# chenruduan/OAReactDiff

Hardware: AMD Instinct MI355X
Metric: denoising_steps_per_sec (higher is better)
Workload: dtype f32; 1 GPU; EGNNDynamics.forward (LEFTNet H=196 R=96 L=6), B=64 reactions/GPU x 3 objects x 23 atoms, complete graph per reaction (N=4416, E=300288), T=1000 sampler step shape; batch_per_gpu=64, atoms_per_object=23, parallelism=replica x1 (no collective), launch=eager

## Files before the change

### oareactdiff_amd/_capi.py

```python
from __future__ import annotations

import ctypes as C
import os

from .build import LIB

OARD_MAX_OBJECTS = 8
ABI_VERSION = 2040
OARD_OK, OARD_EINVAL, OARD_ENOTCOMPLETE, OARD_EHIP, OARD_ENOMEM = 0, -1, -2, -3, -4
ERRORS = {OARD_EINVAL: "invalid argument / unsupported configuration", OARD_ENOTCOMPLETE: "topology is not complete-per-sample",
          OARD_EHIP: "HIP runtime error", OARD_ENOMEM: "workspace too small"}

PREC_GCL_BF16X3, PREC_EQUI_BF16X3, PREC_TRAIN_BF16X3 = 1, 2, 4
TAP_S, TAP_VEC, TAP_EDGE, TAP_POS_FRAME, TAP_DPOS, TAP_HOUT, TAP_LABELS, TAP_NE1 = 1, 2, 3, 4, 5, 6, 7, 8

EXPORTS = ["oard_version", "oard_supported", "oard_param_count", "oard_packed_bytes", "oard_pack_weights",
           "oard_topology_create", "oard_topology_destroy", "oard_topology_num_nodes", "oard_topology_num_edges",
           "oard_topology_num_inner_edges", "oard_topology_num_samples", "oard_topology_check_edge_index",
           "oard_workspace_bytes", "oard_forward", "oard_active_inner_edges", "oard_debug_lin3u_table", "oard_sampler_step", "oard_sampler_step_dev", "oard_tap", "oard_debug_stop_after", "oard_debug_option", "oard_timing_enable", "oard_timing_reset",
           "oard_timing_get",
           "oard_topology_create_parts", "oard_topology_export", "oard_tape_bytes", "oard_tape_entry", "oard_forward_train",
           "oard_packed_bwd_bytes", "oard_pack_weights_bwd", "oard_gcl_backward_dx", "oard_edge_node_sums",
           "oard_equi_backward_dx", "oard_scalarize_backward", "oard_equi_msg_backward", "oard_lin3u_forward", "oard_lin3u_backward", "oard_wgrad_scratch_bytes", "oard_wgrad",
           "oard_train_scratch_bytes", "oard_train_scratch_poison", "oard_train_scratch_entry", "oard_train_tail_backward",
# ... 106 lines not shown
    L.oard_train_stage_backward.restype = ci
    L.oard_nan_replace.argtypes = [cfgp, vp, vp, pvp, pvp, vp]; L.oard_nan_replace.restype = ci
    pf, cf = C.POINTER(C.c_float), C.c_float
    L.oard_loss_prepare.argtypes = [cfgp, vp, pvp, pvp, pvp, pvp, vp, vp, ci, pf, pf, ci, ci, pvp, pvp, vp]; L.oard_loss_prepare.restype = ci
    L.oard_loss_terms.argtypes = [cfgp, vp, pvp, pvp, pvp, pvp, pvp, vp, vp, ci, pf, pf, pf, ci, ci, vp, vp, pvp, vp]; L.oard_loss_terms.restype = ci
    cd = C.c_double
    L.oard_adamw_step.argtypes = [vp, vp, vp, vp, vp, i64, cd, cd, cd, cd, cd, i64, ci, cd, vp]; L.oard_adamw_step.restype = ci
    L.oard_adamw_step_dev.argtypes = [vp, vp, vp, vp, vp, i64, cd, cd, cd, cd, cd, ci, ci, vp, ci, vp, vp, vp, vp]; L.oard_adamw_step_dev.restype = ci
    L.oard_library_stream.argtypes = [ci, pvp]; L.oard_library_stream.restype = ci
    L.oard_graph_create.argtypes = [cfgp, vp, vp, i64, vp, i64, pvp]; L.oard_graph_create.restype = ci
    L.oard_graph_destroy.argtypes = [vp]; L.oard_graph_destroy.restype = None
    L.oard_graph_num_nodes.argtypes = [vp]; L.oard_graph_num_nodes.restype = i64
    L.oard_graph_num_edges.argtypes = [vp]; L.oard_graph_num_edges.restype = i64
    L.oard_graph_object_rows.argtypes = [vp, ci]; L.oard_graph_object_rows.restype = i64
    L.oard_graph_is_complete.argtypes = [vp]; L.oard_graph_is_complete.restype = ci
    L.oard_graph_workspace_bytes.argtypes = [cfgp, vp]; L.oard_graph_workspace_bytes.restype = sz
    L.oard_graph_forward.argtypes = [cfgp, vp, pvp, sz, pvp, vp, ci, vp, pvp, vp, sz, vp, vp]; L.oard_graph_forward.restype = ci
    L.oard_debug_stop_after.argtypes = [C.c_int]; L.oard_debug_stop_after.restype = C.c_int
    L.oard_debug_option.argtypes = [C.c_char_p, C.c_int]; L.oard_debug_option.restype = C.c_int
    L.oard_timing_enable.argtypes = [C.c_int]; L.oard_timing_enable.restype = C.c_int
    L.oard_timing_reset.argtypes = []; L.oard_timing_reset.restype = C.c_int
    L.oard_timing_get.argtypes = [C.c_char_p, C.POINTER(C.c_double), C.POINTER(i64)]; L.oard_timing_get.restype = C.c_int
    for env, opt in (("OARD_GCL_VARIANT", b"gcl_variant"), ("OARD_EQUI_VARIANT", b"equi_variant"),
                     ("OARD_NODE_VARIANT", b"node_variant"), ("OARD_GCL_SKIP", b"gcl_skip"), ("OARD_EQUI_SKIP", b"equi_skip"), ("OARD_EQUI_L0_SKIP", b"equi_l0_skip"), ("OARD_GCL_MSUM", b"gcl_msum"), ("OARD_GCL_PERSIST", b"gcl_persist"), ("OARD_GCL_GRID", b"gcl_grid"), ("OARD_PARTS", b"parts"), ("OARD_SEQUENTIAL", b"sequential"), ("OARD_POISON", b"poison"), ("OARD_AUTO_SMALL", b"auto_small"), ("OARD_AUTO_TINY", b"auto_tiny"), ("OARD_NPB", b"npb"),
                     ("OARD_WGRAD_WGS", b"wgrad_wgs"), ("OARD_WGRAD_LDS", b"wgrad_lds"), ("OARD_WGRAD_T16", b"wgrad_t16"), ("OARD_WGRAD_QUEUE", b"wgrad_queue"), ("OARD_GATE_FOLD", b"gate_fold"), ("OARD_WGRAD_SHAPES", b"wgrad_shapes"), ("OARD_TRAIN_DUAL", b"train_dual"), ("OARD_SMALL_SPLIT", b"small_split"),
                     ("OARD_SKIP_FAMILIES", b"skip_families")):
        if os.environ.get(env) not in (None, ""):
            check(L.oard_debug_option(opt, int(os.environ[env])), f"oard_debug_option({opt.decode()})")
    _lib = L
    return L


def timing_get(family: str):
    ms, n = C.c_double(0.0), C.c_int64(0)
    check(lib().oard_timing_get(family.encode(), C.byref(ms), C.byref(n)), "oard_timing_get")
    return ms.value, n.value
```

### oareactdiff_amd/csrc/oard_hip.hip

```cpp
#include <algorithm>
#include <cmath>
#include <cstdio>
#include <cstring>
#include <map>
#include <string>
#include <vector>
#include <mutex>
#include <chrono>
#include <utility>

#include "oard_kernels.h"
#include "oard_edge_v1.h"
#include "oard_edge_p.h"
#include "oard_wgrad_t16.h"
#include "oard_edge_b3.h"
#ifdef OARD_EXPERIMENTS
#include "oard_edge_fp.h"
#endif
#include "oard_node_v1.h"
#include "oard_edge_small.h"
#include "oard_edge_bwd.h"
#include "oard_node_bwd.h"
#include "oard_rows.h"
#include "oard_inst.h"
// ... 24 lines not shown
        hipEvent_t e; (void)hipEventCreate(&e); return e;
    }
    void flush() {
        for (auto& r : recs) {
            (void)hipEventSynchronize(r.b);
            float ms = 0.f;
            (void)hipEventElapsedTime(&ms, r.a, r.b);
            total_ms[r.fam] += ms; launches[r.fam] += 1;
            pool.push_back(r.a); pool.push_back(r.b);
        }
        recs.clear();
    }
} g_timing;
int g_stop_after = 0;
int g_gcl_variant = 2;
int g_equi_variant = 2;
int g_sequential = 0;
int g_auto_tiny = 8;
int g_auto_small = 4;
int g_npb = 0;
int g_poison = 0;
int g_equi_l0_skip = 1;
int g_gcl_msum = 1;
int g_gcl_msum_taken = 0;
int g_equi_l0_taken = 0;
int g_parts = 0;
int g_small_split = 128;
int g_wgrad_shapes = 3;
int g_wgrad_t16 = 256;
int g_wgrad_lds = 256;
int g_wgrad_wgs = 512;
int g_gcl_persist = 1;
int g_gcl_grid = 0;
int g_equi_skip = 1;
int g_gcl_skip = 1;
int g_node_variant = 1;
int g_skip_families = 0;

struct ScopedLaunch {
    hipStream_t st; hipEvent_t a; int fam; bool on;
    ScopedLaunch(int f, hipStream_t s) : st(s), fam(f), on(g_timing.on) {
        if (on) { a = g_timing.get(); (void)hipEventRecord(a, st); }
    }
    ~ScopedLaunch() {
        if (on) { hipEvent_t b = g_timing.get(); (void)hipEventRecord(b, st); g_timing.recs.push_back({a, b, fam}); }
    }
// ... 198 lines not shown
static thread_local SmallScratch t_small = {nullptr, nullptr};
static WsOff make_ws(const oard_config* c, const TopoDev& td) {
    const RDims d(c->hidden, c->num_radial);
    const size_t N = td.N, E = td.E + 1, A = td.A + 1;
    WsOff w;
    size_t cur = 0;
    auto take = [&](size_t bytes) { size_t o = cur; cur = align_up(cur + bytes, 256); return o; };
    w.pos = take(N * 3 * 4); w.pf64 = take(N * 3 * 8); w.pf32 = take(N * 3 * 4); w.x1 = take(N * 3 * 4);
    w.pp0 = take(N * 4); w.labels = take(N * 4); w.hin = take(N * 16 * 4);
    w.zemb = take(N * d.HP * 4); w.nb = take(N * d.HP * 4); w.s = take(N * d.HP * 4); w.s1 = take(N * d.HP * 4);
    w.ne1 = take(N * 3 * d.HP * 4); w.xh = take(N * d.HP * 4); w.P = take(N * d.HP * 4); w.Q = take(N * d.HP * 4);
    w.xq = take(N * 3 * d.HP * 4); w.vec = take(N * 3 * d.HP * 4); w.vec2 = take(N * 3 * d.HP * 4); w.v2buf = take(N * 3 * d.HP * 4);
    w.sc0 = take(N * d.HP * 4); w.vdot = take(N * d.HP * 4);
    w.geo = take(A * GEO_STRIDE * 4); w.d64 = take(A * 8); w.rbuf = take(A * d.RP * 4);
    w.ew = take(E * d.WP * 4); w.mbuf = take(std::max(E, (size_t)(td.CI + td.CX) + 1) * d.HP * 4);
    w.xmsg = take(A * d.HP * 4); w.vmsg = take(A * 3 * d.HP * 4);
    w.dpos = take(N * 3 * 4); w.hout = take(N * 16 * 4);
    w.al_rows = take(A * 4); w.al_src = take(A * 4); w.al_pre = take(A * 4); w.al_cnt = take((size_t)cdiv((long long)td.A, 256) * 4 + 4); w.al_n = take(4);
    w.d1s = take((size_t)cdiv((long long)td.A, 128) * 8 * d.D1T * 1024);
    w.small_a = w.small_b = 0;
    if (E <= (size_t)OARD_SMALL_MAX_EDGES) {
        w.small_a = take(A * d.D1P * 4);
    }
    w.total = cur;
    return w;
}



template <class K>
int set_lds(K kernel, size_t bytes) {
    HIP_TRY(hipFuncSetAttribute((const void*)kernel, hipFuncAttributeMaxDynamicSharedMemorySize, (int)bytes));
    return OARD_OK;
}

#define LAUNCH_LDS(fam, kern, grid, block, lds, stream, ...) do { \
    static bool attr_done_[64] = {}; \
    int dev_ = 0; (void)hipGetDevice(&dev_); dev_ &= 63; \
    if (!attr_done_[dev_]) { int rc_ = set_lds(kern, lds); if (rc_ != OARD_OK) return rc_; attr_done_[dev_] = true; } \
    ScopedLaunch sl_(fam, stream); if (!((g_skip_families >> (fam)) & 1)) \
    hipLaunchKernelGGL(kern, dim3((unsigned)(grid)), dim3(block), lds, stream, __VA_ARGS__); } while (0)

#define GCL_CASE(id, WV_, GP_) case id: { \
        LAUNCH_LDS(F_GCL_EDGE, (k_gcl_edge_v1<D, WV_, GP_, S1, S3, false>), cdiv(r1 - r0, 16 * WV_), WV_ * 64, \
                   (GclStream<D, GP_>::LDS_BYTES), st, tp, stream, P, Q, u0, c0, r0, r1, ew_in, ew_out, mbuf, GclTape{}); return OARD_OK; }
#define GCL_RING3(TRAIN_, tape_) do { \
// ... 219 lines not shown
    float* xq = (float*)(ws + w.xq); float* vec = slot(w.vec, to.vec_in[0]); float* v2buf = (float*)(ws + w.v2buf);
    float* scal = (float*)(ws + w.sc0); float* vdot = (float*)(ws + w.vdot);
    float* geo = slot(w.geo, to.geo); double* d64 = (double*)(ws + w.d64); float* rbuf = slot(w.rbuf, to.rbuf);
    float* mbuf = (float*)(ws + w.mbuf); float* xmsg = (float*)(ws + w.xmsg);
    float* vmsg = (float*)(ws + w.vmsg); float* dpos = (float*)(ws + w.dpos); float* hout = (float*)(ws + w.hout);
    t_small = (w.small_a && !train) ? SmallScratch{(float*)(ws + w.small_a), (float*)(ws + w.small_b)} : SmallScratch{nullptr, nullptr};
    auto ew_at = [&](int l) -> float* { return train ? (float*)(tape + to.ew[l]) : (float*)(ws + w.ew); };
    float* ew = ew_at(0);
    auto s_at = [&](int l) -> float* { return train ? (float*)(tape + to.s_in[l]) : s; };
    auto s_mid_at = [&](int l) -> float* { return train ? (float*)(tape + to.s_mid[l]) : s; };

    ObjPtrs op;
    memset(&op, 0, sizeof(op));
    for (int k = 0; k < c->n_obj; ++k) {
        op.xh[k] = xh[k]; op.out[k] = out[k]; op.node_nf[k] = c->node_nf[k]; op.enc[k] = po.enc[k]; op.dec[k] = po.dec[k];
    }
    const long long N = tp.N, E = tp.E, A = tp.A;
    const unsigned gN = (unsigned)cdiv(N, 64), gE = (unsigned)cdiv(E, 64), gA = (unsigned)cdiv(A, 64);
    const double cutoff = (double)c->cutoff;
    const int gcl_variant = train ? 2 : g_gcl_variant, equi_variant = train ? 2 : g_equi_variant;
    const int node_variant = train ? 1 : g_node_variant;
    const bool gcl_skip = train || g_gcl_skip;
    const int stop_after = train ? 0 : g_stop_after;
    const bool use_al = !train && g_equi_skip && A > 0 && equi_variant != 0 && node_variant == 1;
    int* al_cnt = (int*)(ws + w.al_cnt);
    const ActList al = use_al ? ActList{(const int*)(ws + w.al_rows), (const int*)(ws + w.al_src), (const int*)(ws + w.al_pre), (const int*)(ws + w.al_n)}
                              : ActList{nullptr, nullptr, nullptr, nullptr};
    if (!use_al) HIP_TRY(hipMemsetAsync(ws + w.al_n, 0xff, sizeof(int), st));
    LAUNCH(F_OTHER, k_prep, cdiv(N, 128), 128, st, tp, op, wb, pos, hin, t, t_scalar, cond,
           c->condition_nf > 0 ? c->condition_nf : 0, c->condition_time, emb);
    LAUNCH(F_INIT, k_geom, tp.n_groups, 64, st, tp, (const float*)pos, cutoff, pf64, pf32, x1, pp0, labels);
    if (!(gcl_skip && gcl_variant != 0) || stop_after == 1)
        LAUNCH(F_INIT, k_fill_edges, std::min<long long>(cdiv((E - A + 1) * (D::WP / 4), 256), 8192), 256, st,
               wb + po.c0row, ew + (size_t)A * D::WP, E - A + 1, D::WP);
    if (A > 0) {
        LAUNCH(F_INIT, k_edge_geo, cdiv(A, 256), 256, st, tp, (const float*)pos, (const double*)pf64, cutoff, geo, d64, use_al ? al_cnt : nullptr);
        if (use_al) LAUNCH(F_INIT, k_active_list, cdiv(A, 256), 256, st, tp, (const float*)geo, (const int*)al_cnt, (int*)al.rows, (int*)al.src, (int*)al.pre, (int*)al.n);
        LAUNCH(F_INIT, k_rbf, cdiv(A * D::RP, 256), 256, st, tp, (const double*)d64, (const float*)geo,
               wb + po.rbf_means, wb + po.rbf_betas, cutoff, rbuf, ew, D::R, D::RP, D::H, D::WP);
    }
    LAUNCH(F_INIT, (k_node_embed<D>), gN, 256, st, tp, wb, po, (const float*)hin, zemb, nb);
    if (A > 0) LAUNCH(F_INIT, (k_radial_lin<D>), gA, 256, st, tp, wb, po, (const float*)rbuf, (const float*)geo, ew);
    constexpr int NW = D::HT <= 16 ? D::HT : 8;
    const unsigned gNb = (unsigned)cdiv(N, tp.npb);
    if (node_variant >= 1) {
        LAUNCH(F_INIT, (k_neighbor_v1<D, NW>), gNb, NW * 64, st, tp, wb, po, (const float*)zemb, (const float*)nb, (const float*)ew, s_at(0), s1);
        LAUNCH(F_INIT, (k_s2v_agg_v1<D, NW>), gNb, NW * 64, st, tp, (const float*)s1, (const float*)ew, (const float*)geo, ne1);
    } else if constexpr (kV0) {
        LAUNCH(F_INIT, (k_neighbor<D>), gN, 256, st, tp, wb, po, (const float*)zemb, (const float*)nb, (const float*)ew, s_at(0), s1);
        LAUNCH(F_INIT, (k_s2v_agg<D>), gN, 256, st, tp, (const float*)s1, (const float*)ew, (const float*)geo, ne1);
    } else return OARD_EINVAL;
    if (A > 0) LAUNCH2(F_INIT, (k_scalarize<D>), gA, (gA * topo->conc <= 2048 ? D::HT : 1), 256, st, tp, wb, po, (const float*)ne1, (const float*)geo, ew);
    HIP_TRY(hipMemsetAsync(vec, 0, (size_t)N * 3 * D::HP * sizeof(float), st));
    if (stop_after == 1) return OARD_OK;

    float* vec2 = (float*)(ws + w.vec2);
    float* vcur = vec;
    float* vnext = vec2;
    const bool msum = !train && g_gcl_msum && E > 0 && gcl_variant == 2 && node_variant == 1 && equi_variant != 0 && tp.npb > 4 &&
                      (tp.CI == 0 || gcl_v1_throughput(c->precision, gcl_variant, topo->conc, tp.CI)) &&
                      (tp.CX == 0 || gcl_v1_throughput(c->precision, gcl_variant, topo->conc, tp.CX));
    g_gcl_msum_taken = msum;
    for (int l = 0; l < c->num_layers; ++l) {
        const LayerOff lo = po.layer[l];
        const bool nv1 = node_variant == 1 && equi_variant != 0;
        const unsigned gN16 = (unsigned)cdiv(N, tp.npb);
        float* ew_in = ew_at(l);
        float* ew_out = ew_at(l + 1);
        if (train) vnext = (float*)(tape + to.vec_in[l + 1]);
// ... 566 lines not shown
        size_t a = 0;
        for (int n = 0; n < N; ++n) {
            const int q = node_sample[n] * n_obj + node_obj[n];
            const int g0 = grp_ptr[q], g1 = grp_ptr[q + 1], s0 = sample_ptr[node_sample[n]];
            act_ptr[n] = (int)a;
            for (int m = g0; m < g1; ++m) if (m != n) {
                act_src[a] = m; act_tgt[a] = n;
                act_edge[a] = edge_ptr[m] + (n - s0) - (n > m ? 1 : 0);
                ++a;
            }
        }
        act_ptr[N] = (int)a;
    }
    std::vector<int> edge_row((size_t)std::max<long long>(E, 1), -1), row_src((size_t)E + 1, 0), row_tgt((size_t)E + 1, 0),
        row_eid((size_t)E + 1, (int)E);
    {
        for (long long a = 0; a < A; ++a) {
            edge_row[act_edge[a]] = (int)a; row_src[a] = act_src[a]; row_tgt[a] = act_tgt[a]; row_eid[a] = act_edge[a];
        }
        long long r = A;
        for (long long e = 0; e < E; ++e)
            if (edge_row[e] < 0) { edge_row[e] = (int)r; row_src[r] = edge_src[e]; row_tgt[r] = edge_tgt[e]; row_eid[r] = (int)e; ++r; }
    }
    std::vector<long long> ref_edge_ptr(N);
    for (int n = 0; n < N; ++n) ref_edge_ptr[n] = ref_ptr_ref[node_ref[n]];
    std::vector<int> col_row, col_info, node_cols((size_t)N * 4, 0);
    long long CI = 0, CX = 0;
    {
        auto pad16 = [&]() { while (col_row.size() % 16) col_row.push_back((int)E); };
        for (int b = 0; b < B; ++b) {
            for (int n = sample_ptr[b]; n < sample_ptr[b + 1]; ++n) {
                const int q = node_sample[n] * n_obj + node_obj[n];
                const int g0 = grp_ptr[q], g1 = grp_ptr[q + 1];
                node_cols[4 * (size_t)n + 0] = (int)col_row.size();
                for (int m = g0; m < g1; ++m) if (m != n) col_row.push_back(act_ptr[m] + (n - g0) - (n > m ? 1 : 0));
                node_cols[4 * (size_t)n + 1] = (int)col_row.size();
            }
            pad16();
        }
        CI = (long long)col_row.size();
        for (int b = 0; b < B; ++b) {
            const int ns = sample_ptr[b + 1] - sample_ptr[b];
            for (int n = sample_ptr[b]; n < sample_ptr[b + 1]; ++n) {
                node_cols[4 * (size_t)n + 2] = (int)col_row.size();
                for (long long e = edge_ptr[n]; e < (long long)edge_ptr[n] + ns - 1; ++e) if (edge_row[e] >= A) col_row.push_back(edge_row[e]);
                node_cols[4 * (size_t)n + 3] = (int)col_row.size();
// ... 3 lines not shown
        CX = (long long)col_row.size() - CI;
        if (CI + CX > 0x7fffffffLL - 256) return OARD_EINVAL;
        if (col_row.empty()) col_row.push_back((int)E);
        col_info.resize(col_row.size() * 4);
        for (size_t k = 0; k < col_row.size(); ++k) {
            const int r = col_row[k];
            col_info[4 * k] = r; col_info[4 * k + 1] = row_src[r]; col_info[4 * k + 2] = row_tgt[r];
            col_info[4 * k + 3] = r == (int)E ? -1 : row_src[r] + 1;
        }
    }

    std::vector<UploadItem> items;
    size_t cur = 0;
    auto add = [&](const void* p, size_t bytes) { UploadItem it{p, bytes, cur}; cur = align_up(cur + bytes, 256); items.push_back(it); return it.off; };
    const size_t o_obj = add(node_obj.data(), N * 4), o_row = add(node_row.data(), N * 4), o_ref = add(node_ref.data(), N * 4),
                 o_tidx = add(node_tidx.data(), N * 4), o_smp = add(node_sample.data(), N * 4),
                 o_sptr = add(sample_ptr.data(), (B + 1) * 4), o_eptr = add(edge_ptr.data(), N * 4),
                 o_esrc = add(edge_src.data(), edge_src.size() * 4), o_etgt = add(edge_tgt.data(), edge_tgt.size() * 4),
                 o_gptr = add(grp_ptr.data(), grp_ptr.size() * 4), o_aptr = add(act_ptr.data(), (N + 1) * 4),
                 o_asrc = add(act_src.data(), act_src.size() * 4), o_atgt = add(act_tgt.data(), act_tgt.size() * 4),
                 o_aedge = add(act_edge.data(), act_edge.size() * 4), o_rptr = add(ref_edge_ptr.data(), N * 8),
                 o_erow = add(edge_row.data(), edge_row.size() * 4), o_rsrc = add(row_src.data(), row_src.size() * 4),
                 o_rtgt = add(row_tgt.data(), row_tgt.size() * 4), o_reid = add(row_eid.data(), row_eid.size() * 4),
                 o_crow = add(col_info.data(), col_info.size() * 4), o_ncol = add(node_cols.data(), node_cols.size() * 4);
    size_t cap = 0;
    char* dev = (char*)pool_alloc(cur, &cap);
    if (!dev) return OARD_EHIP;
    if (int rc = pool_upload(dev, items, cur, &part.stage, &part.stage_cap)) { pool_release(dev, cap, nullptr, 0, false); return rc; }
    part.dev_cap = cap;
    part.dev_block = dev;
    TopoDev& d = part.d;
    d.N = N; d.B = B; d.n_obj = n_obj; d.n_groups = B * n_obj; d.E = E; d.A = A;
    d.node_obj = (const int*)(dev + o_obj); d.node_row = (const int*)(dev + o_row); d.node_ref = (const int*)(dev + o_ref);
    d.node_tidx = (const int*)(dev + o_tidx); d.node_sample = (const int*)(dev + o_smp); d.sample_ptr = (const int*)(dev + o_sptr);
    d.edge_ptr = (const int*)(dev + o_eptr); d.edge_src = (const int*)(dev + o_esrc); d.edge_tgt = (const int*)(dev + o_etgt);
    d.grp_ptr = (const int*)(dev + o_gptr); d.act_ptr = (const int*)(dev + o_aptr); d.act_src = (const int*)(dev + o_asrc);
    d.act_tgt = (const int*)(dev + o_atgt); d.act_edge = (const int*)(dev + o_aedge);
    d.ref_edge_ptr = (const long long*)(dev + o_rptr);
    d.edge_row = (const int*)(dev + o_erow); d.row_src = (const int*)(dev + o_rsrc); d.row_tgt = (const int*)(dev + o_rtgt);
    d.row_eid = (const int*)(dev + o_reid);
    d.CI = CI; d.CX = CX; d.col_info = (const int*)(dev + o_crow); d.node_cols = (const int*)(dev + o_ncol);
    return OARD_OK;
}

int oard_topology_create(const oard_config* c, const int64_t* cm, const int64_t* nfs, int64_t n_nodes,
                         oard_topology** out) {
    return oard_topology_create_parts(c, cm, nfs, n_nodes, g_parts, out);
}

int oard_topology_create_parts(const oard_config* c, const int64_t* cm, const int64_t* nfs, int64_t n_nodes,
                               int parts, oard_topology** out) {
    if (!config_ok(c) || !cm || !nfs || !out || n_nodes < 1 || n_nodes > (1 << 24)) return OARD_EINVAL;
    const int N = (int)n_nodes, n_obj = c->n_obj;
    std::vector<int> obj_start(n_obj + 1, 0);
    for (int i = 0; i < N; ++i) {
        if (nfs[i] < 0 || nfs[i] >= n_obj) return OARD_EINVAL;
        if (i > 0 && nfs[i] < nfs[i - 1]) return OARD_EINVAL;
        obj_start[nfs[i] + 1]++;
    }
    for (int k = 0; k < n_obj; ++k) obj_start[k + 1] += obj_start[k];
    std::vector<int64_t> samples(cm, cm + N);
    std::sort(samples.begin(), samples.end());
    samples.erase(std::unique(samples.begin(), samples.end()), samples.end());
    const int B = (int)samples.size();
// ... 912 lines not shown
                    hipLaunchKernelGGL(k_tap_edges, dim3((unsigned)cdiv(tp.E * d.W, 256)), dim3(256), 0, st, tp,
                                       (const float*)(ws + w.ew), d.WP, d.W, dst);
                break;
            default: return OARD_EINVAL;
        }
    }
    HIP_TRY(hipGetLastError());
    return OARD_OK;
}

int oard_debug_stop_after(int code) { g_stop_after = code; return OARD_OK; }
int oard_debug_option(const char* name, int value) {
    if (!name) return OARD_EINVAL;
    if (!kV0 && value == 0 && (strcmp(name, "gcl_variant") == 0 || strcmp(name, "equi_variant") == 0 || strcmp(name, "node_variant") == 0))
        return OARD_EINVAL;
    if (strcmp(name, "gcl_variant") == 0) { g_gcl_variant = value; return OARD_OK; }
    if (strcmp(name, "equi_variant") == 0) { g_equi_variant = value; return OARD_OK; }
    if (strcmp(name, "node_variant") == 0) { g_node_variant = value; return OARD_OK; }
    if (strcmp(name, "experiments") == 0) return kV0 ? OARD_OK : OARD_EINVAL;
    if (strcmp(name, "gcl_skip") == 0) { g_gcl_skip = value; return OARD_OK; }
    if (strcmp(name, "equi_skip") == 0) { g_equi_skip = value; return OARD_OK; }
    if (strcmp(name, "equi_l0_skip") == 0) { g_equi_l0_skip = value; return OARD_OK; }
    if (strcmp(name, "gcl_msum") == 0) { g_gcl_msum = value; return OARD_OK; }
    if (strcmp(name, "gcl_msum_taken") == 0) return g_gcl_msum_taken ? OARD_OK : OARD_EINVAL;
    if (strcmp(name, "equi_l0_taken") == 0) return g_equi_l0_taken ? OARD_OK : OARD_EINVAL;
    if (strcmp(name, "gcl_persist") == 0) { g_gcl_persist = value; return OARD_OK; }
    if (strcmp(name, "gcl_grid") == 0) { g_gcl_grid = value; return OARD_OK; }
    if (strcmp(name, "skip_families") == 0) { g_skip_families = value; return OARD_OK; }
    if (strcmp(name, "parts") == 0) { g_parts = value; return OARD_OK; }
    if (strcmp(name, "sequential") == 0) { g_sequential = value; return OARD_OK; }
    if (strcmp(name, "poison") == 0) { g_poison = value; return OARD_OK; }
    if (strcmp(name, "auto_small") == 0) { g_auto_small = value; return OARD_OK; }
    if (strcmp(name, "auto_tiny") == 0) { g_auto_tiny = value; return OARD_OK; }
    if (strcmp(name, "npb") == 0) { g_npb = value; return OARD_OK; }
    if (strcmp(name, "wgrad_wgs") == 0) { g_wgrad_wgs = value; return OARD_OK; }
    if (strcmp(name, "wgrad_t16") == 0) { g_wgrad_t16 = value; return OARD_OK; }
    if (strcmp(name, "wgrad_queue") == 0) { g_wgrad_queue = value; return OARD_OK; }
    if (strcmp(name, "gate_fold") == 0) { g_gate_fold = value; return OARD_OK; }
    if (strcmp(name, "wgrad_lds") == 0) { g_wgrad_lds = value; return OARD_OK; }
    if (strcmp(name, "wgrad_shapes") == 0) { g_wgrad_shapes = value & 3; return OARD_OK; }
    if (strcmp(name, "train_dual") == 0) { g_train_dual = value; return OARD_OK; }
    if (strcmp(name, "small_split") == 0) { g_small_split = value; return OARD_OK; }
    return OARD_EINVAL;
}
#ifdef OARD_PHASE_PROBE
int oard_debug_probe_read(unsigned long long* out8) {
// ... 40 lines not shown
```

### oareactdiff_amd/csrc/oard_kernels.h

```cpp
#pragma once
#include "oard_engine.h"
#include "oard_layout.h"

#define GEO_STRIDE 12
#define EPSF 1e-6

struct ColId {
    int lane, g, col;
    bool valid;
    long long c;
};
OARD_DEV ColId col_id(long long ncols, bool& wave_live) {
    ColId id;
    id.lane = threadIdx.x & 63;
    id.g = id.lane >> 4;
    const long long cb = (long long)blockIdx.x * 4 + (threadIdx.x >> 6);
    wave_live = cb * 16 < ncols;
    const long long c = cb * 16 + (id.lane & 15);
    id.valid = c < ncols;
    id.c = id.valid ? c : (ncols > 0 ? ncols - 1 : 0);
    id.col = (int)id.c;
    return id;
}

// ... 474 lines not shown
    if (on) { rows[off] = (int)a; src[off] = tp.act_src[a]; }
    if (a == tp.A - 1) { const int tot = off + (on ? 1 : 0); pre[tp.A] = tot; *n_act = tot; }
}
OARD_KERNEL __global__ void k_rbf(TopoDev tp, const double* __restrict__ d64, const float* __restrict__ geo,
                      const float* __restrict__ means, const float* __restrict__ betas, double cutoff,
                      float* __restrict__ rbuf, float* __restrict__ ew, int R, int RP, int H, int WP) {
    const long long i = (long long)blockIdx.x * blockDim.x + threadIdx.x;
    if (i >= tp.A * RP) return;
    const long long a = i / RP;
    const int k = (int)(i % RP);
    float v = 0.f;
    if (k < R) {
        const double d = d64[a], m = (double)geo[a * GEO_STRIDE + 11];
        double rb = 0.5 * (cos(d * M_PI / cutoff) + 1.0);
        rb = d < cutoff ? rb : 0.0;
        const double q = exp(-d) - (double)means[k];
        v = (float)(rb * exp(-(double)betas[k] * q * q) * m);
        ew[(size_t)a * WP + 3 * H + k] = v;
        if (k == 0)
            for (int c = 3 * H + R; c < WP; ++c) ew[(size_t)a * WP + c] = 0.f;
    }
    rbuf[i] = v;
}

OARD_KERNEL __global__ void k_fill_edges(const float* __restrict__ c0, float* __restrict__ ew, long long E, int WP) {
    const int per = WP / 4;
    const long long total = E * per;
    for (long long i = (long long)blockIdx.x * blockDim.x + threadIdx.x; i < total; i += (long long)gridDim.x * blockDim.x)
        st_f4(ew + i * 4, ld_f4(c0 + (i % per) * 4));
}

template <class D>
__global__ __launch_bounds__(256) void k_node_embed(TopoDev tp, const float* __restrict__ wb, PackOff po,
                                                    const float* __restrict__ hin, float* __restrict__ zemb,
                                                    float* __restrict__ nb) {
    bool live; const ColId id = col_id(tp.N, live);
    if (!live) return;
    f4 in[1] = {ld_blk(hin, id.c, 16, 0, id.lane)};
    f4 v[D::HT];
#pragma unroll
    for (int t = 0; t < D::HT; ++t) {
        f4 z = dense_tile<1>(wb + po.emb, t, in, id.lane, ld_vec(wb + po.emb_b, t, id.lane));
        if (id.valid) st_blk(zemb, id.c, D::HP, t, id.lane, z);
        v[t] = dense_tile<1>(wb + po.nbemb, t, in, id.lane, ld_vec(wb + po.nbemb_b, t, id.lane));
    }
    layer_norm<D::HT, D::H, false>(v, nullptr, nullptr, id.lane);
    if (id.valid)
#pragma unroll
        for (int t = 0; t < D::HT; ++t) st_blk(nb, id.c, D::HP, t, id.lane, v[t]);
}

template <class D>
__global__ __launch_bounds__(256) void k_radial_lin(TopoDev tp, const float* __restrict__ wb, PackOff po,
                                                    const float* __restrict__ rbuf, const float* __restrict__ geo,
                                                    float* __restrict__ ew) {
    bool live; const ColId id = col_id(tp.A, live);
    if (!live) return;
    f4 rb[D::RB];
#pragma unroll
    for (int b = 0; b < D::RB; ++b) rb[b] = ld_blk(rbuf, id.c, D::RP, b, id.lane);
    f4 h1[D::HT];
    dense_regs<D::RB, D::HT, true, true>(wb + po.rl0, wb + po.rl0_b, rb, h1, id.lane);
    const float env = geo[id.c * GEO_STRIDE + 1];
    const size_t row = (size_t)id.c * D::WP + 2 * D::H;
#pragma unroll
    for (int t = 0; t < D::HT; ++t) {
        f4 f = dense_tile<D::HT>(wb + po.rl2, t, h1, id.lane, ld_vec(wb + po.rl2_b, t, id.lane));
        if (id.valid && 16 * t + 4 * id.g < D::H) st_f4(ew + row + 16 * t + 4 * id.g, f * env);
    }
}

template <class D>
__global__ __launch_bounds__(256) void k_neighbor(TopoDev tp, const float* __restrict__ wb, PackOff po,
                                                  const float* __restrict__ zemb, const float* __restrict__ nb,
                                                  const float* __restrict__ ew, float* __restrict__ s,
                                                  float* __restrict__ s1) {
    bool live; const ColId id = col_id(tp.N, live);
    if (!live) return;
    const int n = id.col, smp = tp.node_sample[n], s0 = tp.sample_ptr[smp], ns = tp.sample_ptr[smp + 1] - s0;
    f4 acc[D::HT];
#pragma unroll
    for (int t = 0; t < D::HT; ++t) acc[t] = f4zero();
    const int mx = wave_max(ns);
    for (int k = 0; k < mx; ++k) {
        const int m = s0 + k;
        if (k < ns && m != n) {
            const int r = tp.edge_row[tp.edge_ptr[m] + (n - s0) - (n > m ? 1 : 0)];
            const float* frow = (r < tp.A ? ew + (size_t)r * D::WP : wb + po.c0row) + 2 * D::H;
#pragma unroll
            for (int t = 0; t < D::HT; ++t)
                if (16 * t + 4 * id.g < D::H)
// ... 448 lines not shown
```

### oareactdiff_amd/csrc/oard_layout.h

```cpp
#pragma once
#include <hip/hip_runtime.h>
#include <stdint.h>
#include <stddef.h>
#include "../../include/oard.h"

#define OARD_MAX_LAYERS 16
#define OARD_MAX_GROUP 1024

template <int H_, int R_>
struct Dims {
    static constexpr int H = H_, R = R_;
    static constexpr int HT = (H + 15) / 16, HP = HT * 16;
    static constexpr int W = 3 * H + R, WB = (W + 15) / 16, WP = WB * 16;
    static constexpr int RB = (R + 15) / 16, RP = RB * 16;
    static constexpr int H2 = H / 2, PB = (H2 + 15) / 16, PP = PB * 16;
    static constexpr int D1T = (3 * H + 15) / 16, D1P = D1T * 16;
    static constexpr int H4 = H / 4;
    static_assert(H % 4 == 0 && R % 4 == 0, "feature widths must be multiples of 4");
};

struct RDims {
    int H, R, HT, HP, W, WB, WP, RB, RP, H2, PB, PP, D1T, D1P, H4;
    explicit RDims(int h, int r) {
        H = h; R = r; HT = (H + 15) / 16; HP = HT * 16; W = 3 * H + R; WB = (W + 15) / 16; WP = WB * 16;
// ... 25 lines not shown
    size_t u0;
    size_t rbf_means, rbf_betas;
    size_t enc[OARD_MAX_OBJECTS], dec[OARD_MAX_OBJECTS];
    LayerOff layer[OARD_MAX_LAYERS];
    size_t total;
    int signed_scal;
};

struct TopoDev {
    int N, B, n_obj, n_groups;
    int npb;
    long long E, A;
    const int *node_obj, *node_row, *node_ref, *node_tidx, *node_sample, *sample_ptr;
    const int *edge_ptr, *edge_src, *edge_tgt;
    const int *edge_row;
    const int *row_src, *row_tgt;
    const int *row_eid;
    const int *grp_ptr;
    const int *act_ptr, *act_src, *act_tgt, *act_edge;
    const long long *ref_edge_ptr;
    long long CI, CX;
    const int *col_info;
    const int *node_cols;
};

struct ActList {
    const int* rows;
    const int* src;
    const int* pre;
    const int* n;
};

#define OARD_MAX_PARTS 8
struct TopoPart {
    TopoDev d;
    void* dev_block = nullptr;
    size_t dev_cap = 0;
    void* stage = nullptr;
    size_t stage_cap = 0;
    size_t ws_off = 0;
    int conc = 1;
    mutable size_t vec_final = 0;
};
struct oard_topology {
    int device = 0;
    int n_parts = 0;
// ... 3 lines not shown
    int max_group = 0, max_ns = 0;
    int obj_start[OARD_MAX_OBJECTS + 1] = {};
    hipStream_t side[OARD_MAX_PARTS] = {};
    hipEvent_t ev_fork = nullptr, ev_join[OARD_MAX_PARTS] = {};
    void* ref_block = nullptr;
    size_t ref_cap = 0;
    void* ref_stage = nullptr;
    size_t ref_stage_cap = 0;
    hipEvent_t ready = nullptr;
    mutable hipStream_t used_on[4] = {};
    mutable int n_used = 0;
    mutable bool used_many = false;
    const int *ref_sample = nullptr, *ref_rank = nullptr;
    const long long* ref_ptr = nullptr;
    int N_ref = 0;
};

struct WsOff {
    size_t pos, pf64, pf32, x1, pp0, labels, hin, zemb, nb, s, s1, ne1, xh, P, Q, xq, vec, vec2, v2buf, sc0, vdot,
        geo, d64, rbuf, ew, mbuf, xmsg, vmsg, dpos, hout, total;
    size_t al_rows, al_src, al_pre, al_cnt, al_n;
    size_t d1s;
    size_t small_a, small_b;
};
```

### oareactdiff_amd/csrc/oard_node_v1.h

```cpp
#pragma once
#include "oard_kernels.h"

OARD_DEV f4 lds_blk(const float* v, int b, int lane) { return *reinterpret_cast<const f4*>(v + b * 256 + lane * 4); }
OARD_DEV void lds_st(float* v, int t, int lane, f4 x) { *reinterpret_cast<f4*>(v + t * 256 + lane * 4) = x; }

#ifndef OARD_NODE_PF
#define OARD_NODE_PF 13
#endif
template <int KB>
OARD_DEV f4 dense_tile_lds(const float* __restrict__ wp, int t, const float* in, int lane, f4 init) {
    const float* base = wp + ((size_t)t * KB * 64 + lane) * 4;
    f4 c0 = init, c1 = f4zero();
    constexpr int G = OARD_NODE_PF;
#pragma unroll
    for (int b0 = 0; b0 < KB; b0 += G) {
        f4 a[G];
#pragma unroll
        for (int i = 0; i < G; ++i)
            if (b0 + i < KB) a[i] = ld_f4(base + (size_t)(b0 + i) * 256);
        __builtin_amdgcn_sched_barrier(0);
#pragma unroll
        for (int i = 0; i < G; ++i)
            if (b0 + i < KB) {
                const f4 x = lds_blk(in, b0 + i, lane);
// ... 657 lines not shown
        for (int i = 0; i < TPW; ++i) {
            const int t = min(nb.wave + i * WAVES, HT - 1);
#pragma unroll
            for (int k = 0; k < 3; ++k) { job[3 * i + k] = tile_job<HT>(wb + lo.xv2, k * HT + t, hx); acc[3 * i + k] = f4zero(); }
        }
        dense_seq<HT, 3 * TPW>(job, nb.lane, acc);
#pragma unroll
        for (int i = 0; i < TPW; ++i) {
            const int t = nb.wave + i * WAVES;
            if (t < HT && nb.valid) {
                const f4 a = acc[3 * i], b = acc[3 * i + 1], c = acc[3 * i + 2];
                st_blk(s_out, n, D::HP, t, nb.lane, lds_blk(in, t, nb.lane) + (a + b + vdk[i]) * inv_sqrt2);
#pragma unroll
                for (int x = 0; x < 3; ++x)
                    st_blk(vec_out, (size_t)n * 3 + x, D::HP, t, nb.lane,
                           lds_blk(vx + x * HT * 256, t, nb.lane) + c * v2k[i][x]);
            }
        }
    }
    TL(0);
    TL_END();
}

template <class D, int WAVES>
__global__ __launch_bounds__(WAVES * 64) void k_neighbor_v1(TopoDev tp, const float* __restrict__ wb, PackOff po,
                                                            const float* __restrict__ zemb, const float* __restrict__ nbe,
                                                            const float* __restrict__ ew, float* __restrict__ s,
                                                            float* __restrict__ s1) {
    constexpr int HT = D::HT, TPW = (HT + WAVES - 1) / WAVES;
    __shared__ __attribute__((aligned(16))) float sm[2 * HT * 256];
    float* sv = sm;
    float* yv = sm + HT * 256;
    const NodeBlk nb = node_blk(tp.N, tp.npb);
    const int n = nb.n, smp = tp.node_sample[n], s0 = tp.sample_ptr[smp];
    const int ns = nb.valid ? tp.sample_ptr[smp + 1] - s0 : 0;
    const int mx = wave_max(ns);
    const int self = n - s0;
    const float* c0f = wb + po.c0row + 2 * D::H;
    for (int t = nb.wave; t < HT; t += WAVES) {
        f4 acc = f4zero();
        const bool fok = 16 * t + 4 * nb.g < D::H;
        const int fo = 16 * t + 4 * nb.g;
        for (int k = 0; k < mx; k += 4) {
            int r[4];
#pragma unroll
            for (int i = 0; i < 4; ++i) {
                const int kk = min(k + i, max(ns - 1, 0)), m = s0 + kk;
                r[i] = kk == self ? -1 : tp.edge_row[tp.edge_ptr[m] + self - (self > kk ? 1 : 0)];
            }
            f4 f[4], x[4];
#pragma unroll
            for (int i = 0; i < 4; ++i) {
                const int kk = min(k + i, max(ns - 1, 0));
                const float* frow = (r[i] >= 0 && r[i] < tp.A) ? ew + (size_t)r[i] * D::WP + 2 * D::H : c0f;
                f[i] = fok ? ld_f4(frow + fo) : f4zero();
                x[i] = ld_blk(nbe, s0 + kk, D::HP, t, nb.lane);
            }
#pragma unroll
            for (int i = 0; i < 4; ++i)
                if (k + i < ns && r[i] >= 0) acc += f[i] * x[i];
        }
        acc += ld_blk(zemb, n, D::HP, t, nb.lane);
        lds_st(sv, t, nb.lane, acc);
        if (nb.valid) st_blk(s, n, D::HP, t, nb.lane, acc);
    }
// ... 181 lines not shown
```

Before: 3694 reaction-steps/s.

## Exploit edge symmetry in RBF/radial init and factor cross-object neighbor sums

```diff
diff --git a/oareactdiff_amd/_capi.py b/oareactdiff_amd/_capi.py
--- a/oareactdiff_amd/_capi.py
+++ b/oareactdiff_amd/_capi.py
@@ -152,7 +152,7 @@
     L.oard_timing_reset.argtypes = []; L.oard_timing_reset.restype = C.c_int
     L.oard_timing_get.argtypes = [C.c_char_p, C.POINTER(C.c_double), C.POINTER(i64)]; L.oard_timing_get.restype = C.c_int
     for env, opt in (("OARD_GCL_VARIANT", b"gcl_variant"), ("OARD_EQUI_VARIANT", b"equi_variant"),
-                     ("OARD_NODE_VARIANT", b"node_variant"), ("OARD_GCL_SKIP", b"gcl_skip"), ("OARD_EQUI_SKIP", b"equi_skip"), ("OARD_EQUI_L0_SKIP", b"equi_l0_skip"), ("OARD_GCL_MSUM", b"gcl_msum"), ("OARD_GCL_PERSIST", b"gcl_persist"), ("OARD_GCL_GRID", b"gcl_grid"), ("OARD_PARTS", b"parts"), ("OARD_SEQUENTIAL", b"sequential"), ("OARD_POISON", b"poison"), ("OARD_AUTO_SMALL", b"auto_small"), ("OARD_AUTO_TINY", b"auto_tiny"), ("OARD_NPB", b"npb"),
+                     ("OARD_NODE_VARIANT", b"node_variant"), ("OARD_GCL_SKIP", b"gcl_skip"), ("OARD_EQUI_SKIP", b"equi_skip"), ("OARD_EQUI_L0_SKIP", b"equi_l0_skip"), ("OARD_GCL_MSUM", b"gcl_msum"), ("OARD_INIT_V2", b"init_v2"), ("OARD_GCL_PERSIST", b"gcl_persist"), ("OARD_GCL_GRID", b"gcl_grid"), ("OARD_PARTS", b"parts"), ("OARD_SEQUENTIAL", b"sequential"), ("OARD_POISON", b"poison"), ("OARD_AUTO_SMALL", b"auto_small"), ("OARD_AUTO_TINY", b"auto_tiny"), ("OARD_NPB", b"npb"),
                      ("OARD_WGRAD_WGS", b"wgrad_wgs"), ("OARD_WGRAD_LDS", b"wgrad_lds"), ("OARD_WGRAD_T16", b"wgrad_t16"), ("OARD_WGRAD_QUEUE", b"wgrad_queue"), ("OARD_GATE_FOLD", b"gate_fold"), ("OARD_WGRAD_SHAPES", b"wgrad_shapes"), ("OARD_TRAIN_DUAL", b"train_dual"), ("OARD_SMALL_SPLIT", b"small_split"),
                      ("OARD_SKIP_FAMILIES", b"skip_families")):
         if os.environ.get(env) not in (None, ""):
diff --git a/oareactdiff_amd/csrc/oard_hip.hip b/oareactdiff_amd/csrc/oard_hip.hip
--- a/oareactdiff_amd/csrc/oard_hip.hip
+++ b/oareactdiff_amd/csrc/oard_hip.hip
@@ -70,6 +70,7 @@
 int g_poison = 0;
 int g_equi_l0_skip = 1;
 int g_gcl_msum = 1;
+int g_init_v2 = 1;
 int g_gcl_msum_taken = 0;
 int g_equi_l0_taken = 0;
 int g_parts = 0;
@@ -314,6 +315,7 @@
     if (E <= (size_t)OARD_SMALL_MAX_EDGES) {
         w.small_a = take(A * d.D1P * 4);
     }
+    w.objsum = take((size_t)std::max(td.n_groups, 1) * d.HP * 4);
     w.total = cur;
     return w;
 }
@@ -579,6 +581,7 @@
     const int node_variant = train ? 1 : g_node_variant;
     const bool gcl_skip = train || g_gcl_skip;
     const int stop_after = train ? 0 : g_stop_after;
+    const bool v2_pairs = g_init_v2 == 1 || g_init_v2 == 2, v2_objsum = g_init_v2 == 1 || g_init_v2 == 4;
     const bool use_al = !train && g_equi_skip && A > 0 && equi_variant != 0 && node_variant == 1;
     int* al_cnt = (int*)(ws + w.al_cnt);
     const ActList al = use_al ? ActList{(const int*)(ws + w.al_rows), (const int*)(ws + w.al_src), (const int*)(ws + w.al_pre), (const int*)(ws + w.al_n)}
@@ -593,15 +596,28 @@
     if (A > 0) {
         LAUNCH(F_INIT, k_edge_geo, cdiv(A, 256), 256, st, tp, (const float*)pos, (const double*)pf64, cutoff, geo, d64, use_al ? al_cnt : nullptr);
         if (use_al) LAUNCH(F_INIT, k_active_list, cdiv(A, 256), 256, st, tp, (const float*)geo, (const int*)al_cnt, (int*)al.rows, (int*)al.src, (int*)al.pre, (int*)al.n);
-        LAUNCH(F_INIT, k_rbf, cdiv(A * D::RP, 256), 256, st, tp, (const double*)d64, (const float*)geo,
-               wb + po.rbf_means, wb + po.rbf_betas, cutoff, rbuf, ew, D::R, D::RP, D::H, D::WP);
+        if (v2_pairs)
+            LAUNCH(F_INIT, k_rbf_pairs, cdiv(tp.AP * D::RP, 256), 256, st, tp, (const double*)d64, (const float*)geo,
+                   wb + po.rbf_means, wb + po.rbf_betas, cutoff, rbuf, ew, D::R, D::RP, D::H, D::WP);
+        else
+            LAUNCH(F_INIT, k_rbf, cdiv(A * D::RP, 256), 256, st, tp, (const double*)d64, (const float*)geo,
+                   wb + po.rbf_means, wb + po.rbf_betas, cutoff, rbuf, ew, D::R, D::RP, D::H, D::WP);
     }
     LAUNCH(F_INIT, (k_node_embed<D>), gN, 256, st, tp, wb, po, (const float*)hin, zemb, nb);
-    if (A > 0) LAUNCH(F_INIT, (k_radial_lin<D>), gA, 256, st, tp, wb, po, (const float*)rbuf, (const float*)geo, ew);
+    if (A > 0) {
+        if (v2_pairs) LAUNCH(F_INIT, (k_radial_lin_pairs<D>), cdiv(tp.AP, 64), 256, st, tp, wb, po, (const float*)rbuf, (const float*)geo, ew);
+        else LAUNCH(F_INIT, (k_radial_lin<D>), gA, 256, st, tp, wb, po, (const float*)rbuf, (const float*)geo, ew);
+    }
     constexpr int NW = D::HT <= 16 ? D::HT : 8;
     const unsigned gNb = (unsigned)cdiv(N, tp.npb);
     if (node_variant >= 1) {
-        LAUNCH(F_INIT, (k_neighbor_v1<D, NW>), gNb, NW * 64, st, tp, wb, po, (const float*)zemb, (const float*)nb, (const float*)ew, s_at(0), s1);
+        if (v2_objsum) {
+            float* objsum = (float*)(ws + w.objsum);
+            LAUNCH(F_INIT, (k_nb_objsum<D>), tp.n_groups, 64, st, tp, (const float*)nb, objsum);
+            LAUNCH(F_INIT, (k_neighbor_v1<D, NW, true>), gNb, NW * 64, st, tp, wb, po, (const float*)zemb, (const float*)nb, (const float*)ew, s_at(0), s1, (const float*)objsum);
+        } else {
+            LAUNCH(F_INIT, (k_neighbor_v1<D, NW>), gNb, NW * 64, st, tp, wb, po, (const float*)zemb, (const float*)nb, (const float*)ew, s_at(0), s1, (const float*)nullptr);
+        }
         LAUNCH(F_INIT, (k_s2v_agg_v1<D, NW>), gNb, NW * 64, st, tp, (const float*)s1, (const float*)ew, (const float*)geo, ne1);
     } else if constexpr (kV0) {
         LAUNCH(F_INIT, (k_neighbor<D>), gN, 256, st, tp, wb, po, (const float*)zemb, (const float*)nb, (const float*)ew, s_at(0), s1);
@@ -1214,6 +1230,14 @@
         for (long long e = 0; e < E; ++e)
             if (edge_row[e] < 0) { edge_row[e] = (int)r; row_src[r] = edge_src[e]; row_tgt[r] = edge_tgt[e]; row_eid[r] = (int)e; ++r; }
     }
+    std::vector<int> pair_rows;
+    pair_rows.reserve((size_t)A + 2);
+    for (long long a = 0; a < A; ++a) {
+        const int m = act_src[a], n = act_tgt[a];
+        if (m > n) { pair_rows.push_back((int)a); pair_rows.push_back(act_ptr[m] + (n - grp_ptr[node_sample[n] * n_obj + node_obj[n]])); }
+    }
+    const long long AP = (long long)pair_rows.size() / 2;
+    pair_rows.push_back(0); pair_rows.push_back(0);
     std::vector<long long> ref_edge_ptr(N);
     for (int n = 0; n < N; ++n) ref_edge_ptr[n] = ref_ptr_ref[node_ref[n]];
     std::vector<int> col_row, col_info, node_cols((size_t)N * 4, 0);
@@ -1263,7 +1287,8 @@
                  o_aedge = add(act_edge.data(), act_edge.size() * 4), o_rptr = add(ref_edge_ptr.data(), N * 8),
                  o_erow = add(edge_row.data(), edge_row.size() * 4), o_rsrc = add(row_src.data(), row_src.size() * 4),
                  o_rtgt = add(row_tgt.data(), row_tgt.size() * 4), o_reid = add(row_eid.data(), row_eid.size() * 4),
-                 o_crow = add(col_info.data(), col_info.size() * 4), o_ncol = add(node_cols.data(), node_cols.size() * 4);
+                 o_crow = add(col_info.data(), col_info.size() * 4), o_ncol = add(node_cols.data(), node_cols.size() * 4),
+                 o_pair = add(pair_rows.data(), pair_rows.size() * 4);
     size_t cap = 0;
     char* dev = (char*)pool_alloc(cur, &cap);
     if (!dev) return OARD_EHIP;
@@ -1281,6 +1306,7 @@
     d.edge_row = (const int*)(dev + o_erow); d.row_src = (const int*)(dev + o_rsrc); d.row_tgt = (const int*)(dev + o_rtgt);
     d.row_eid = (const int*)(dev + o_reid);
     d.CI = CI; d.CX = CX; d.col_info = (const int*)(dev + o_crow); d.node_cols = (const int*)(dev + o_ncol);
+    d.AP = AP; d.pair_rows = (const int*)(dev + o_pair);
     return OARD_OK;
 }
 
@@ -2239,6 +2265,7 @@
     if (strcmp(name, "equi_skip") == 0) { g_equi_skip = value; return OARD_OK; }
     if (strcmp(name, "equi_l0_skip") == 0) { g_equi_l0_skip = value; return OARD_OK; }
     if (strcmp(name, "gcl_msum") == 0) { g_gcl_msum = value; return OARD_OK; }
+    if (strcmp(name, "init_v2") == 0) { g_init_v2 = value; return OARD_OK; }
     if (strcmp(name, "gcl_msum_taken") == 0) return g_gcl_msum_taken ? OARD_OK : OARD_EINVAL;
     if (strcmp(name, "equi_l0_taken") == 0) return g_equi_l0_taken ? OARD_OK : OARD_EINVAL;
     if (strcmp(name, "gcl_persist") == 0) { g_gcl_persist = value; return OARD_OK; }
diff --git a/oareactdiff_amd/csrc/oard_kernels.h b/oareactdiff_amd/csrc/oard_kernels.h
--- a/oareactdiff_amd/csrc/oard_kernels.h
+++ b/oareactdiff_amd/csrc/oard_kernels.h
@@ -520,6 +520,29 @@
     }
     rbuf[i] = v;
 }
+OARD_KERNEL __global__ void k_rbf_pairs(TopoDev tp, const double* __restrict__ d64, const float* __restrict__ geo,
+                            const float* __restrict__ means, const float* __restrict__ betas, double cutoff,
+                            float* __restrict__ rbuf, float* __restrict__ ew, int R, int RP, int H, int WP) {
+    const long long i = (long long)blockIdx.x * blockDim.x + threadIdx.x;
+    if (i >= tp.AP * RP) return;
+    const long long p = i / RP;
+    const int k = (int)(i % RP);
+    const long long a = tp.pair_rows[2 * p], b = tp.pair_rows[2 * p + 1];
+    float v = 0.f;
+    if (k < R) {
+        const double d = d64[a], m = (double)geo[a * GEO_STRIDE + 11];
+        double rb = 0.5 * (cos(d * M_PI / cutoff) + 1.0);
+        rb = d < cutoff ? rb : 0.0;
+        const double q = exp(-d) - (double)means[k];
+        v = (float)(rb * exp(-(double)betas[k] * q * q) * m);
+        ew[(size_t)a * WP + 3 * H + k] = v;
+        ew[(size_t)b * WP + 3 * H + k] = v;
+        if (k == 0)
+            for (int c = 3 * H + R; c < WP; ++c) { ew[(size_t)a * WP + c] = 0.f; ew[(size_t)b * WP + c] = 0.f; }
+    }
+    rbuf[(size_t)a * RP + k] = v;
+    rbuf[(size_t)b * RP + k] = v;
+}
 
 OARD_KERNEL __global__ void k_fill_edges(const float* __restrict__ c0, float* __restrict__ ew, long long E, int WP) {
     const int per = WP / 4;
@@ -565,6 +588,30 @@
     for (int t = 0; t < D::HT; ++t) {
         f4 f = dense_tile<D::HT>(wb + po.rl2, t, h1, id.lane, ld_vec(wb + po.rl2_b, t, id.lane));
         if (id.valid && 16 * t + 4 * id.g < D::H) st_f4(ew + row + 16 * t + 4 * id.g, f * env);
+    }
+}
+
+template <class D>
+__global__ __launch_bounds__(256) void k_radial_lin_pairs(TopoDev tp, const float* __restrict__ wb, PackOff po,
+                                                          const float* __restrict__ rbuf, const float* __restrict__ geo,
+                                                          float* __restrict__ ew) {
+    bool live; const ColId id = col_id(tp.AP, live);
+    if (!live) return;
+    const size_t a = (size_t)tp.pair_rows[2 * id.c], b = (size_t)tp.pair_rows[2 * id.c + 1];
+    f4 rb[D::RB];
+#pragma unroll
+    for (int k = 0; k < D::RB; ++k) rb[k] = ld_blk(rbuf, a, D::RP, k, id.lane);
+    f4 h1[D::HT];
+    dense_regs<D::RB, D::HT, true, true>(wb + po.rl0, wb + po.rl0_b, rb, h1, id.lane);
+    const float env = geo[a * GEO_STRIDE + 1];
+    const size_t row_a = a * D::WP + 2 * D::H, row_b = b * D::WP + 2 * D::H;
+#pragma unroll
+    for (int t = 0; t < D::HT; ++t) {
+        f4 f = dense_tile<D::HT>(wb + po.rl2, t, h1, id.lane, ld_vec(wb + po.rl2_b, t, id.lane));
+        if (id.valid && 16 * t + 4 * id.g < D::H) {
+            st_f4(ew + row_a + 16 * t + 4 * id.g, f * env);
+            st_f4(ew + row_b + 16 * t + 4 * id.g, f * env);
+        }
     }
 }
 
diff --git a/oareactdiff_amd/csrc/oard_layout.h b/oareactdiff_amd/csrc/oard_layout.h
--- a/oareactdiff_amd/csrc/oard_layout.h
+++ b/oareactdiff_amd/csrc/oard_layout.h
@@ -71,6 +71,8 @@
     long long CI, CX;
     const int *col_info;
     const int *node_cols;
+    long long AP;
+    const int *pair_rows;
 };
 
 struct ActList {
@@ -120,4 +122,5 @@
     size_t al_rows, al_src, al_pre, al_cnt, al_n;
     size_t d1s;
     size_t small_a, small_b;
+    size_t objsum;
 };
diff --git a/oareactdiff_amd/csrc/oard_node_v1.h b/oareactdiff_amd/csrc/oard_node_v1.h
--- a/oareactdiff_amd/csrc/oard_node_v1.h
+++ b/oareactdiff_amd/csrc/oard_node_v1.h
@@ -703,11 +703,22 @@
     TL_END();
 }
 
-template <class D, int WAVES>
+template <class D>
+__global__ __launch_bounds__(64) void k_nb_objsum(TopoDev tp, const float* __restrict__ nbe, float* __restrict__ objsum) {
+    static_assert(D::HP <= 256, "one wave per row, four channels per lane");
+    const int q = blockIdx.x, ch = 4 * threadIdx.x;
+    if (ch >= D::HP) return;
+    const int g0 = tp.grp_ptr[q], g1 = tp.grp_ptr[q + 1];
+    f4 acc = f4zero();
+    for (int m = g0; m < g1; ++m) acc += ld_f4(nbe + (size_t)m * D::HP + ch);
+    st_f4(objsum + (size_t)q * D::HP + ch, acc);
+}
+
+template <class D, int WAVES, bool OBJSUM = false>
 __global__ __launch_bounds__(WAVES * 64) void k_neighbor_v1(TopoDev tp, const float* __restrict__ wb, PackOff po,
                                                             const float* __restrict__ zemb, const float* __restrict__ nbe,
                                                             const float* __restrict__ ew, float* __restrict__ s,
-                                                            float* __restrict__ s1) {
+                                                            float* __restrict__ s1, const float* __restrict__ objsum = nullptr) {
     constexpr int HT = D::HT, TPW = (HT + WAVES - 1) / WAVES;
     __shared__ __attribute__((aligned(16))) float sm[2 * HT * 256];
     float* sv = sm;
@@ -718,10 +729,31 @@
     const int mx = wave_max(ns);
     const int self = n - s0;
     const float* c0f = wb + po.c0row + 2 * D::H;
+    const int a0 = tp.act_ptr[n], cnt = nb.valid ? tp.act_ptr[n + 1] - a0 : 0, own = tp.node_obj[n];
+    const int mxi = OBJSUM ? wave_max(cnt) : 0;
+    const long long a_hi = max(tp.A - 1, 0LL);
     for (int t = nb.wave; t < HT; t += WAVES) {
         f4 acc = f4zero();
         const bool fok = 16 * t + 4 * nb.g < D::H;
         const int fo = 16 * t + 4 * nb.g;
+        if constexpr (OBJSUM) {
+            for (int k = 0; k < mxi; k += 4) {
+                f4 f[4], x[4];
+#pragma unroll
+                for (int i = 0; i < 4; ++i) {
+                    const size_t a = (size_t)min((long long)a0 + min(k + i, max(cnt - 1, 0)), a_hi);
+                    f[i] = fok ? ld_f4(ew + a * D::WP + 2 * D::H + fo) : f4zero();
+                    x[i] = ld_blk(nbe, tp.act_src[a], D::HP, t, nb.lane);
+                }
+#pragma unroll
+                for (int i = 0; i < 4; ++i)
+                    if (k + i < cnt) acc += f[i] * x[i];
+            }
+            f4 ext = f4zero();
+            for (int o = 0; o < tp.n_obj; ++o)
+                if (o != own) ext += ld_blk(objsum, (size_t)smp * tp.n_obj + o, D::HP, t, nb.lane);
+            if (fok) acc += ld_f4(c0f + fo) * ext;
+        } else
         for (int k = 0; k < mx; k += 4) {
             int r[4];
 #pragma unroll
```

Result: no change. 3704 reaction-steps/s (median of 6 runs) (+0.3%).
